# zhexin1904/gtsam_personal

Hardware: AMD Instinct MI355X
Metric: LM iterations/sec (higher is better)
Workload: dtype f64; 1 GPU; synthetic BAL 1000 cameras / 100000 points / 1000002 factors (GeneralSFMFactor<Cal3Bundler> + 2 priors), seed 42, METIS ordering (Ordering::Metis of the reference, fixture-carried permutation), LM legacy defaults; ordering=metis, cameras=1000, points=100000, factors=1000002, fronts=100001, parallelism=single GPU

## Files before the change

### gtsam_personal_amd/_lib.py

```python
from __future__ import annotations

import ctypes as ct
import os

_HERE = os.path.dirname(os.path.abspath(__file__))
LIB_PATH = os.path.join(_HERE, "liblmgpu.so")

LMGPU_OK, LMGPU_INDETERMINATE, LMGPU_INVALID, LMGPU_HIP_ERROR = 0, 1, 2, 3


class lmgpu_config(ct.Structure):
    _fields_ = [("device", ct.c_int32), ("rank", ct.c_int32), ("world_size", ct.c_int32), ("flags", ct.c_int32)]


class lmgpu_lm_params(ct.Structure):
    _fields_ = [
        ("maxIterations", ct.c_int32),
        ("relativeErrorTol", ct.c_double), ("absoluteErrorTol", ct.c_double), ("errorTol", ct.c_double),
        ("lambdaInitial", ct.c_double), ("lambdaFactor", ct.c_double), ("lambdaUpperBound", ct.c_double), ("lambdaLowerBound", ct.c_double),
        ("minModelFidelity", ct.c_double),
        ("diagonalDamping", ct.c_int32), ("useFixedLambdaFactor", ct.c_int32),
        ("minDiagonal", ct.c_double), ("maxDiagonal", ct.c_double),
    ]

# ... 119 lines not shown
    "lmgpu_ncg_optimize": (ct.c_int, [_H, ct.POINTER(lmgpu_ncg_params), ct.POINTER(lmgpu_lm_state)]),
    "lmgpu_ncg_get_trace": (ct.c_int, [_H, ct.c_int32, _D]),
    "lmgpu_ncg_host_waits": (ct.c_int, [_H]),
    "lmgpu_init_pose3_create": (ct.c_int, [ct.POINTER(lmgpu_config), ct.POINTER(_H)]),
    "lmgpu_init_pose3_destroy": (ct.c_int, [_H]),
    "lmgpu_init_pose3_last_error": (ct.c_char_p, [_H]),
    "lmgpu_init_pose3_add_factors": (ct.c_int, [_H, ct.c_int32, ct.c_int32, _I, ct.POINTER(ct.c_uint64), _D, ct.c_int32, _D]),
    "lmgpu_init_pose3_finalize": (ct.c_int, [_H, ct.c_int32, ct.POINTER(ct.c_uint64)]),
    "lmgpu_init_pose3_num_poses": (ct.c_int, [_H]),
    "lmgpu_init_pose3_num_factors": (ct.c_int, [_H]),
    "lmgpu_init_pose3_get_slots": (ct.c_int, [_H, ct.POINTER(ct.c_uint64)]),
    "lmgpu_init_pose3_handle": (ct.c_void_p, [_H, ct.c_int32]),
    "lmgpu_init_pose3_orientations_chordal": (ct.c_int, [_H, _D]),
    "lmgpu_init_pose3_closest_rotations": (ct.c_int, [ct.c_int32, ct.c_int32, _D, _D]),
    "lmgpu_init_pose3_orientations_gradient": (ct.c_int, [_H, _D, ct.c_int32, ct.c_int32, _D, _I, _D]),
    "lmgpu_init_pose3_compute_poses": (ct.c_int, [_H, _D, ct.c_int32, _D, ct.POINTER(lmgpu_lm_state)]),
    "lmgpu_init_pose3_initialize": (ct.c_int, [_H, _D, ct.c_int32, _D]),
    "lmgpu_set_kernel_timing": (ct.c_int, [_H, ct.c_int32]),
    "lmgpu_get_kernel_times": (ct.c_int, [_H, _D, _D, ct.POINTER(ct.c_int64)]),
    "lmgpu_get_jacobian": (ct.c_int, [_H, ct.c_int32, _D, _I, _I]),
    "lmgpu_get_jacobians": (ct.c_int, [_H, _I, _I, _I, _I, ct.POINTER(ct.c_int64), _D]),
    "lmgpu_num_fronts": (ct.c_int, [_H]),
    "lmgpu_front_info": (ct.c_int, [_H, ct.c_int32, _I]),
    "lmgpu_get_front": (ct.c_int, [_H, ct.c_int32, _I, _D]),
    "lmgpu_comm_unique_id": (ct.c_int, [ct.c_char_p]),
    "lmgpu_comm_init": (ct.c_int, [_H, ct.c_char_p]),
    "lmgpu_marginal_covariance": (ct.c_int, [_H, ct.c_int32, _D]),
    "lmgpu_joint_marginal_covariance": (ct.c_int, [_H, ct.c_int32, _I, _D]),
    "lmgpu_selftest_chain_schedule": (ct.c_int, [ct.c_int, ct.c_int, ct.c_int, ct.c_int, ct.c_int]),
    "lmgpu_selftest_dense_schedule": (ct.c_int, [ct.c_int, ct.c_int, ct.c_int, ct.c_uint, ct.c_int, _I]),
    "lmgpu_selftest_dogleg_step": (ct.c_int, [ct.c_int, _D, _D]),
    "lmgpu_bt_products": (ct.c_int, [_H, _D, ct.c_double, _D, _D]),
    "lmgpu_isam2_create": (ct.c_int, [ct.POINTER(lmgpu_config), ct.c_void_p, ct.c_void_p, ct.c_void_p, ct.POINTER(_H)]),
    "lmgpu_isam2_destroy": (ct.c_int, [_H]),
    "lmgpu_isam2_last_error": (ct.c_char_p, [_H]),
    "lmgpu_isam2_last_failed_key": (ct.c_uint64, [_H]),
    "lmgpu_isam2_add_variables": (ct.c_int, [_H, ct.c_int32, ct.POINTER(ct.c_uint64), _I, _D]),
    "lmgpu_isam2_add_factors": (ct.c_int, [_H, ct.c_int32, ct.c_int32, ct.POINTER(ct.c_uint64), _D, ct.c_int32, _D]),
    "lmgpu_isam2_add_factors_robust": (ct.c_int, [_H, ct.c_int32, ct.c_int32, ct.POINTER(ct.c_uint64), _D, ct.c_int32, _D, ct.c_int32, ct.c_double]),
    "lmgpu_isam2_update": (ct.c_int, [_H, ct.c_int32, ct.c_void_p]),
    "lmgpu_isam2_update_with": (ct.c_int, [_H, ct.c_void_p, ct.c_void_p]),
    "lmgpu_isam2_set_relinearize_thresholds": (ct.c_int, [_H, ct.c_int32, ct.c_char_p, _I, _D]),
    "lmgpu_isam2_set_partial_relinearization_check": (ct.c_int, [_H, ct.c_int32]),
    "lmgpu_isam2_set_dogleg": (ct.c_int, [_H, ct.c_double, ct.c_double, ct.c_int32]),
    "lmgpu_isam2_get_dogleg_delta": (ct.c_double, [_H]),
    "lmgpu_isam2_set_evaluate_nonlinear_error": (ct.c_int, [_H, ct.c_int32]),
# ... 80 lines not shown
```

### gtsam_personal_amd/csrc/kernels_front.hpp

```cpp
#pragma once
#include <hip/hip_runtime.h>

#include "kernels_factors.hpp"

namespace lmgpu {

struct FrontFac {
  int32_t fac;
  int32_t c0, c1, c2;
};
struct ChildRef {
  int64_t u_off;
  int32_t ld, m;
  int32_t map_begin;
  int32_t pad;
};
struct FrontDesc {
  int32_t n, nf;
  int32_t fac_begin, fac_count;
  int32_t child_begin, child_count;
  int32_t fx_begin;
  int32_t sx_begin;
  int64_t rsd_off;
  int64_t u_off;
// ... 1064 lines not shown
  __shared__ int s_ticket, s_ok;
  const int tid = threadIdx.x, lane = tid & 63;
  if (tid == 0) s_ticket = (int)atomicAdd(ticket, 1u);
  __syncthreads();
  const int fi = list[seg_end - 1 - s_ticket];
  const FrontDesc F = fronts[fi];
  const int ns = F.n - F.nf - 1;
  const int so = sxoff[F.sx_begin + max(min(tid, ns - 1), 0)], fo = fxoff[F.fx_begin + min(tid, F.nf - 1)];
  ldsb_stage(F, pool, Ls, tid);
  bool bad, timed_out = false;
  const double* y = ldsb_solve_core<true>(F, Ls, ns > 0 ? so : fo, delta, &bad, &timed_out);
  if (tid < F.nf)
    __hip_atomic_store((unsigned long long*)(delta + fo), (unsigned long long)__double_as_longlong(y[tid]), __ATOMIC_RELAXED, __HIP_MEMORY_SCOPE_AGENT);
  if (bad && lane == 0) atomicMin(status, F.id);
  if (timed_out) atomicExch(status + 1, 1 + F.id);
  (void)s_ok;
  (void)parent_of;
  (void)pos_of;
  (void)done;
  (void)lane;
}

}
```

### gtsam_personal_amd/csrc/lmgpu.hip

```cpp
#include <hip/hip_runtime.h>
#include <rccl/rccl.h>

#include <algorithm>
#include <chrono>
#include <cmath>
#include <cstdio>
#include <cstdlib>
#include <cstring>
#include <condition_variable>
#include <limits>
#include <mutex>
#include <string>
#include <map>
#include <vector>

#include "../../include/lmgpu.h"
#include "kernels_dense.hpp"
#include "kernels_potrf.hpp"
#include "kernels_step.hpp"
#include "dense_schedule.hpp"
#include "dogleg_step.hpp"
#include "kernels_batched.hpp"
#include "kernels_level.hpp"
#include "kernels_bayes.hpp"
// ... 33 lines not shown
  } while (0)

namespace {

struct Bucket {
  int type = 0, n = 0, noise_kind = 0;
  int robust = 0;
  double robust_k = 0.0;
  std::vector<int32_t> graph_index, slots;
  std::vector<double> meas, noise;
  int rows = 0, cols = 0;
  int n_loc = 0;
  std::vector<int32_t> loc_of;
  int64_t joff = 0;
  int32_t* d_vidx = nullptr;
  double* d_meas = nullptr;
  double* d_noise = nullptr;
  int32_t* d_epos = nullptr;
};

struct LevelWork {
  int list_begin = 0, list_count = 0;
  int lds_nf_max = 0;
  int lds_rsd_max = 0;
  int bin_begin[16] = {0};
  int bin_srows[16] = {0};
  int bin_jcap[16] = {0};
  int64_t pack_off[16] = {0};
  int pack_stride[16] = {0};
  std::vector<int> hbm;
  int small_begin = 0, small_count = 0;
  int bsd_begin = 0, bsd_count = 0;
  int med_begin = 0, med_count = 0, med_max_fac = 0, med_max_child = 0, med_max_nf = 0, med_max_cols = 0, med_max_n = 0;
  int fuse_task_begin = 0, fuse_task_count = 0, fuse_nmax = 0, fuse_jcap = 0, fuse_threads = 0;
};

struct KTimer {
  bool on = false;
  bool dominant_only = false;
  std::vector<hipEvent_t> pool;
  struct Rec {
    int cat, e0, e1, launches;
  };
  std::vector<Rec> recs;
  int used = 0;
  double ms[LMGPU_KT_NUM] = {0}, work[LMGPU_KT_NUM] = {0};
  long long cnt[LMGPU_KT_NUM] = {0};
  int grab() {
    if (used == (int)pool.size()) {
      hipEvent_t e;
      (void)hipEventCreate(&e);
      pool.push_back(e);
// ... 106 lines not shown
  int chain_split_pct = 60;
  bool chain_merge = true;
  int chain_far_pct = 50;
  double* d_lambda = nullptr;
  bool merge_backsub = false;
  struct ElimSeg {
    int lvl_lo, lvl_hi, nmax, jcap, threads;
  };
  std::vector<ElimSeg> elim_segs;
  std::vector<int> elim_seg_of;
  bool merge_elim = false;
  FillUpper* d_fill_upper = nullptr;
  int n_fill_upper = 0;
  bool fuse_levels = false;
  LevelTask* d_level_tasks = nullptr;
  LevelSync* d_level_sync = nullptr;
  int n_level_sync = 0;
  int32_t *d_bs_parent = nullptr, *d_bs_pos = nullptr;
  char* d_leafpack = nullptr;
  unsigned int* d_bs_done = nullptr;
  bool use_graph = false;
  int eager_solves = 0;
  hipGraphExec_t solve_graph[2] = {nullptr, nullptr};
  bool no_wide16 = false;
  int wide16_max = 256;
  bool bsd_ticket = false;
  bool no_tail = false;
  bool no_chain = false;
  int chain_forms = 0;
  unsigned int* d_pflags = nullptr;
  int pflags_panels = 0;
  unsigned int* bs_flags = nullptr;
  double* pool = nullptr;
  size_t pool_doubles = 0;
  double* vals[2][kNumVarTypes] = {};
  double* saved[kNumVarTypes] = {};
  int cur = 0;
  int32_t* type_xoff[kNumVarTypes] = {};
  double *delta = nullptr, *dampw = nullptr, *hdiag = nullptr, *ebuf0 = nullptr, *ebuf1 = nullptr, *partial = nullptr, *dscal = nullptr,
         *ywork = nullptr;
  int* d_status = nullptr;
  double* h_scal = nullptr;
  int* h_status = nullptr;
  FacDesc* d_fd = nullptr;
  FrontDesc* d_fronts = nullptr;
  FrontFac* d_ffac = nullptr;
// ... 494 lines not shown
    if (fused) {
      const MedLevel ML{(const MedFront*)(h->d_med_fronts + L.med_begin)};
      const size_t lds = std::max<size_t>(kLdsFrontExtra - (size_t)(LDSF_JCAP - L.fuse_jcap) * 8 + 64 + (size_t)L.fuse_nmax * L.fuse_nmax * sizeof(double),
                                          (size_t)DIAG_LDS_BYTES);
      unsigned int* ticket = h->d_bs_done + h->h_fronts.size() + li;
      const int kt = h->kt.begin(LMGPU_KT_PANEL, s);
      const bool wide = L.fuse_threads == 1024;
      auto* kernel = wide ? level_fused_kernel<1024> : level_fused_kernel<256>;
      hipLaunchKernelGGL(kernel, dim3(L.fuse_task_count), dim3(wide ? 1024 : 256), lds, s, (const LevelTask*)(h->d_level_tasks + L.fuse_task_begin), ticket,
                         (const int32_t*)h->d_lists, (const FrontDesc*)h->d_fronts, (const FrontFac*)h->d_ffac, (const FacDesc*)h->d_fd,
                         (const ChildRef*)h->d_childs, (const int32_t*)h->d_cmap, (const int32_t*)h->d_fxoff, h->pool, lambda_v, lambda_p,
                         (const double*)h->dampw, h->d_status, L.fuse_nmax, L.fuse_jcap, (const double*)h->gex_active, ML, (const int32_t*)h->d_rowptr,
                         (const RowSrc*)h->d_rowsrc, h->inv16_med, h->d_level_sync + L.med_begin);
      h->kt.end(kt, s);
    }
    for (int b = 0; b < kNumBins && seg == -1 && !fused; b++) {
      const int cnt = L.bin_begin[b + 1] - L.bin_begin[b];
      if (cnt == 0) continue;
      const int nmax = kBinN[b % 6], srows = L.bin_srows[b];
      const int threads = (b >= 6 || b % 6 == 0) ? 64 : (b % 6 == 1 ? 128 : 256);
      const int jcap = L.bin_jcap[b];
      const size_t lds = kLdsFrontExtra - (size_t)(LDSF_JCAP - jcap) * 8 + 64 + (size_t)srows * nmax * sizeof(double);
      const int kt = h->kt.begin(LMGPU_KT_LDS_FRONT, s);
      const bool wide16 = b >= 3 && b < 6 && cnt <= h->wide16_max && !h->no_wide16;
      auto* kernel = lds_front_kernel<false, 1024>;
      if (!wide16) kernel = b < 6 ? lds_front_kernel<false> : lds_front_kernel<true>;
      hipLaunchKernelGGL(kernel, dim3(cnt), dim3(wide16 ? 1024 : threads), lds, s,
                         (const int32_t*)(h->d_lists + L.list_begin + L.bin_begin[b]), (const FrontDesc*)h->d_fronts,
                         (const FrontFac*)h->d_ffac, (const FacDesc*)h->d_fd, (const ChildRef*)h->d_childs, (const int32_t*)h->d_cmap,
                         (const int32_t*)h->d_fxoff, h->pool, lambda_v, lambda_p, (const double*)h->dampw, h->d_status, nmax, srows, h->d_gcorner, jcap,
                         (const double*)h->gex_active, (const char*)(h->d_leafpack && L.pack_stride[b] ? h->d_leafpack + L.pack_off[b] : nullptr),
                         L.pack_stride[b]);
      h->kt.end(kt, s);
    }
    if (L.med_count > 0 && !fused) {
      const MedLevel ML{(const MedFront*)(h->d_med_fronts + L.med_begin)};
      const unsigned cnt = (unsigned)L.med_count;
      int ktm = h->kt.begin(LMGPU_KT_HBM_ASSEMBLE, s);
      if (L.med_max_fac > 0 || L.med_max_child > 0)
        hipLaunchKernelGGL(med_assemble_rows_kernel, dim3((L.med_max_n + 3) / 4, cnt), dim3(256), 0, s, ML, (const int32_t*)h->d_rowptr, (const RowSrc*)h->d_rowsrc, (const ChildRef*)h->d_childs, (const int32_t*)h->d_cmap,
                           (const FrontFac*)h->d_ffac, (const FacDesc*)h->d_fd, h->pool, (const int32_t*)h->d_fxoff, lambda_v, lambda_p,
                           (const double*)h->dampw, (const double*)h->gex_active);
      else
        hipLaunchKernelGGL(med_damp_kernel, dim3((L.med_max_nf + 255) / 256, cnt), dim3(256), 0, s, ML, (const int32_t*)h->d_fxoff, h->pool, lambda_v,
                           lambda_p, (const double*)h->dampw, (const double*)h->gex_active);
      h->kt.end(ktm, s);
// ... 145 lines not shown
          }
          case DENSE_TAIL: {
            const int ktt = h->kt.begin(LMGPU_KT_PANEL, s);
            hipLaunchKernelGGL(front_tail_kernel, dim3(1), dim3(256), TAIL_LDS_BYTES, s, A, ld, F.n, F.nf, k0, kb, F.id, h->d_status,
                               h->inv16 + (size_t)(i + 1) * 4096);
            h->kt.end(ktt, s, st.flop);
            break;
          }
          case DENSE_ADD_CHUNK:
          case DENSE_WAIT_CHUNK: {
            const int rcc = st.kind == DENSE_ADD_CHUNK ? add_chunk(h, A, Asm, F.n, ld, st.chunk) : wait_chunk(h, Asm, F.n, ld, st.chunk);
            if (rcc) return rcc;
            break;
          }
        }
      }
      if (run_launches > 0) h->kt.end(kt_run, s, run_flop, run_launches);
    }
  }
  HIPCHECK(hipGetLastError());
  return LMGPU_OK;
}

static bool level_lds_class(const lmgpu_handle* h, int l, int* nmax, int* jcap, int* threads) {
  const int kMergeCap = 160;
  const LevelWork& L = h->levels[l];
  if (L.list_count == 0 || L.list_count > kMergeCap || L.bin_begin[kNumBins] != L.bin_begin[6]) return false;
  int top = -1, jc = 96, cnt_top = 0;
  for (int b = 0; b < 6; b++)
    if (L.bin_begin[b + 1] > L.bin_begin[b]) {
      top = b;
      cnt_top = L.bin_begin[b + 1] - L.bin_begin[b];
      jc = std::max(jc, L.bin_jcap[b]);
    }
  *nmax = kBinN[top];
  *jcap = jc;
  const bool wide16 = top >= 3 && cnt_top <= h->wide16_max && !h->no_wide16;
  *threads = wide16 ? 1024 : (top == 0 ? 64 : 256);
  return true;
}

int do_backsub(lmgpu_handle* h) {
  hipStream_t s = h->stream;
  if (h->cfg.world_size > 1) HIPCHECK(hipMemsetAsync(h->delta, 0, h->ntot * sizeof(double), s));
  const bool merge = h->merge_backsub && h->cfg.world_size == 1 && !(h->cfg.flags & LMGPU_FLAG_SPLIT_ROOT);
  const bool no_bsd_runs = dev_switch("LMGPU_NO_BSD_RUNS") != nullptr;
  const int NFR = (int)h->h_fronts.size();
  if (h->n_fill_backsub < 0 || h->fill_backsub_merge != (int)merge) {
    std::vector<FillChunk> fills;
    if (merge) {
      add_fill(fills, h->d_bs_done, (size_t)(NFR + h->levels.size() + 1) * sizeof(unsigned int), 0u);
      add_fill(fills, h->delta, h->ntot * sizeof(double), 0xffffffffu);
    }
    if (h->bsd_x_count > 0) {
      add_fill(fills, h->d_bsd_x, h->bsd_x_count * sizeof(double), 0xffffffffu);
      add_fill(fills, h->d_bsd_ticket, h->levels.size() * sizeof(unsigned int), 0u);
    }
    if (h->d_fill_backsub) {
      HIPCHECK(hipStreamSynchronize(s));
      (void)hipFree(h->d_fill_backsub);
      h->d_fill_backsub = nullptr;
    }
    h->n_fill_backsub = (int)fills.size();
    h->fill_backsub_merge = (int)merge;
    if (!fills.empty()) {
      const int rcu = upload(h, &h->d_fill_backsub, fills);
      if (rcu) return rcu;
    }
  }
  if (h->n_fill_backsub > 0) hipLaunchKernelGGL(fill_chunks_kernel, dim3(h->n_fill_backsub), dim3(256), 0, s, (const FillChunk*)h->d_fill_backsub);
  int seg_hi = -1, seg_lo = -1;
  auto run_level = [&](const LevelWork& L) {
    if (L.lds_nf_max > LDSB_SMALL_NF) {
      hipLaunchKernelGGL(lds_backsub_wide_kernel, dim3(L.list_count), dim3(256), (size_t)(L.lds_rsd_max + LDSB_TAIL) * sizeof(double), s,
                         (const int32_t*)(h->d_lists + L.list_begin), L.list_count, (const FrontDesc*)h->d_fronts, (const int32_t*)h->d_fxoff,
                         (const int32_t*)h->d_sxoff, (const double*)h->pool, h->delta, h->d_status);
    } else {
      hipLaunchKernelGGL(lds_backsub_kernel, dim3((L.list_count + 3) / 4), dim3(256), 0, s, (const int32_t*)(h->d_lists + L.list_begin),
                         L.list_count, (const FrontDesc*)h->d_fronts, (const int32_t*)h->d_fxoff, (const int32_t*)h->d_sxoff,
                         (const double*)h->pool, h->delta, h->d_status);
    }
  };
  auto flush_segment = [&]() -> int {
    if (seg_hi < 0) return LMGPU_OK;
    const int kt = h->kt.begin(LMGPU_KT_BACKSUB_LDS, s);
    if (seg_hi == seg_lo) {
      run_level(h->levels[seg_hi]);
    } else {
      const int b = h->levels[seg_lo].list_begin, e = h->levels[seg_hi].list_begin + h->levels[seg_hi].list_count;
      int rsdmax = 0;
      for (int l = seg_lo; l <= seg_hi; l++) rsdmax = std::max(rsdmax, h->levels[l].lds_rsd_max);
      hipLaunchKernelGGL(lds_backsub_merged_kernel, dim3(e - b), dim3(256), (size_t)(rsdmax + LDSB_TAIL) * sizeof(double), s, (const int32_t*)h->d_lists, b, e,
                         (const FrontDesc*)h->d_fronts, (const int32_t*)h->d_fxoff, (const int32_t*)h->d_sxoff, (const double*)h->pool, h->delta,
                         h->d_status, (const int32_t*)h->d_bs_parent, (const int32_t*)h->d_bs_pos, h->d_bs_done, h->d_bs_done + NFR + seg_hi);
    }
    h->kt.end(kt, s);
    seg_hi = seg_lo = -1;
    return LMGPU_OK;
  };
// ... 732 lines not shown
    const Front& fr = P.fronts[fi];
    if (rep[fi]) continue;
    h->front_owner[fi] = (fr.parent < 0 || rep[fr.parent]) ? top_owner[fi] : h->front_owner[fr.parent];
  }
  for (int fi = 0; fi < NF; fi++) h->front_active[fi] = rep[fi] || h->front_owner[fi] == R;
}

}

extern "C" {

int lmgpu_create(const lmgpu_config* cfg, lmgpu_handle** out) {
  if (!cfg || !out) return LMGPU_INVALID;
  lmgpu_handle* h = new lmgpu_handle();
  h->cfg = *cfg;
  if (h->cfg.world_size < 1) h->cfg.world_size = 1;
  h->device = cfg->device;
  h->two_launch_panel = dev_switch("LMGPU_PANEL_2L") != nullptr;
  h->no_fuse = dev_switch("LMGPU_NO_FUSE") != nullptr;
  h->no_chain = dev_switch("LMGPU_NO_CHAIN") != nullptr;
  h->chain_forms = (dev_switch("LMGPU_CHAIN_FENCED_TILES") ? CHAIN_FORM_FENCED_TILES : 0) | (dev_switch("LMGPU_CHAIN_PREREAD") ? CHAIN_FORM_PREREAD : 0);
  h->no_tail = dev_switch("LMGPU_NO_TAIL") != nullptr;
  h->no_wide16 = dev_switch("LMGPU_NO_WIDE16") != nullptr;
  if (const char* e = dev_switch("LMGPU_WIDE16_MAX")) h->wide16_max = atoi(e);
  h->bsd_ticket = dev_switch("LMGPU_BSD_TICKET") != nullptr;
  h->no_gather_write = dev_switch("LMGPU_NO_GATHER_WRITE") != nullptr;
  h->schur_split_diag = dev_switch("LMGPU_SCHUR_SPLIT_DIAG") != nullptr;
  h->pcg_fused = dev_switch("LMGPU_PCG_FUSED") != nullptr;
  if (dev_switch("LMGPU_NO_MERGE")) h->chain_merge = false;
  if (const char* e = dev_switch("LMGPU_CHAIN_SPLIT")) h->chain_split_pct = std::max(0, std::min(100, atoi(e)));
  if (const char* e = dev_switch("LMGPU_CHAIN_FAR")) h->chain_far_pct = std::max(10, std::min(100, atoi(e)));
  *out = h;
  if (h->device >= 0) {
    HIPCHECK(hipSetDevice(h->device));
    {
      hipDeviceProp_t prop;
      HIPCHECK(hipGetDeviceProperties(&prop, h->device));
      h->num_cus = prop.multiProcessorCount;
    }
    HIPCHECK(hipStreamCreate(&h->stream));
    {
      int prio_lo = 0, prio_hi = 0;
      HIPCHECK(hipDeviceGetStreamPriorityRange(&prio_lo, &prio_hi));
      HIPCHECK(hipStreamCreateWithPriority(&h->comm_stream, hipStreamNonBlocking, prio_hi));
    }
    HIPCHECK(hipEventCreateWithFlags(&h->asm_ev, hipEventDisableTiming));
// ... 593 lines not shown
  std::vector<int32_t> lists;
  for (int l = 0; l < P.n_levels; l++) {
    LevelWork& L = h->levels[l];
    L.list_begin = (int)lists.size();
    int c = 0;
    for (int b = 0; b < kNumBins; b++) {
      L.bin_begin[b] = c;
      L.bin_srows[b] = kBinN[b % 6];
      if (b >= 6) {
        int mx = 1;
        for (int fi : byLevelBin[l][b]) mx = std::max(mx, P.fronts[fi].nf);
        L.bin_srows[b] = mx;
      }
      int jc = 96;
      for (int fi : byLevelBin[l][b]) {
        int tot = 0;
        for (int32_t f : P.fronts[fi].factors) tot += fd[h->fac_local[f]].rows * (fd[h->fac_local[f]].d0 + fd[h->fac_local[f]].d1 + fd[h->fac_local[f]].d2 + 1);
        jc = std::max(jc, std::min(tot, LDSF_JCAP));
      }
      L.bin_jcap[b] = (jc + 7) & ~7;
      for (int fi : byLevelBin[l][b]) {
        lists.push_back(fi);
        L.lds_nf_max = std::max(L.lds_nf_max, (int)P.fronts[fi].nf);
        L.lds_rsd_max = std::max(L.lds_rsd_max, (int)P.fronts[fi].nf * ((int)P.fronts[fi].n | 1));
      }
      c += (int)byLevelBin[l][b].size();
    }
    L.bin_begin[kNumBins] = c;
    L.list_count = c;
  }
  {
    h->elim_segs.clear();
    h->elim_seg_of.assign(P.n_levels, -1);
    auto level_class = [&](int l, int* nmax, int* jcap, int* threads) { return level_lds_class(h, l, nmax, jcap, threads); };
    int l = 0;
    while (l < P.n_levels) {
      int nmax, jcap, threads;
      if (!level_class(l, &nmax, &jcap, &threads)) {
        l++;
        continue;
      }
      lmgpu_handle::ElimSeg E{l, l, nmax, jcap, threads};
      while (E.lvl_hi + 1 < P.n_levels && h->levels[E.lvl_hi].hbm.empty()) {
        int n2, j2, t2;
        if (!level_class(E.lvl_hi + 1, &n2, &j2, &t2) || (t2 == 1024) != (E.threads == 1024)) break;
        E.lvl_hi++;
        E.nmax = std::max(E.nmax, n2);
        E.jcap = std::max(E.jcap, j2);
        E.threads = std::max(E.threads, t2);
      }
      if (E.lvl_hi > E.lvl_lo) {
        h->elim_seg_of[E.lvl_lo] = (int)h->elim_segs.size();
        for (int q = E.lvl_lo + 1; q <= E.lvl_hi; q++) h->elim_seg_of[q] = -2;
// ... 1183 lines not shown
  std::vector<std::vector<double>> jb(h->buckets.size());
  for (size_t k = 0; k < h->buckets.size(); k++) {
    const Bucket& b = h->buckets[k];
    jb[k].resize((size_t)b.n_loc * b.rows * b.cols);
    if (b.n_loc) HIPCHECK(hipMemcpy(jb[k].data(), h->pool + b.joff, jb[k].size() * sizeof(double), hipMemcpyDeviceToHost));
  }
  off = 0;
  for (int i = 0; i < NFAC; i++) {
    const FactorRef& f = h->plan.factors[i];
    const Bucket& b = h->buckets[f.bucket];
    const size_t sz = (size_t)b.rows * b.cols;
    if (b.loc_of[f.idx] < 0) {
      h->err = "lmgpu_get_jacobians: a factor lives on another rank";
      return LMGPU_INVALID;
    }
    std::memcpy(out + off, jb[f.bucket].data() + (size_t)b.loc_of[f.idx] * sz, sz * sizeof(double));
    off += (int64_t)sz;
  }
  return LMGPU_OK;
}

int lmgpu_num_fronts(const lmgpu_handle* h) { return (h && h->finalized) ? (int)h->plan.fronts.size() : -1; }

int lmgpu_front_info(const lmgpu_handle* h, int32_t front, int32_t* info) {
  if (!h || !h->finalized || front < 0 || front >= (int)h->plan.fronts.size() || !info) return LMGPU_INVALID;
  const Front& fr = h->plan.fronts[front];
  info[0] = (int)fr.vars.size();
  info[1] = fr.n_frontal_vars;
  info[2] = fr.nf;
  info[3] = fr.n;
  info[4] = fr.parent;
  info[5] = fr.cls;
  info[6] = h->front_owner[front];
  info[7] = fr.level;
  return LMGPU_OK;
}

int lmgpu_get_front(lmgpu_handle* h, int32_t front, int32_t* slots, double* RSd) {
  if (!h) return LMGPU_INVALID;
  if (!h->finalized || front < 0 || front >= (int)h->plan.fronts.size()) {
    h->err = "lmgpu_get_front: refused (!h->finalized || front < 0 || front >= (int)h->plan.fronts.size())";
    return LMGPU_INVALID;
  }
  const Front& fr = h->plan.fronts[front];
  if (slots) std::memcpy(slots, fr.vars.data(), fr.vars.size() * sizeof(int32_t));
  if (RSd) {
// ... 382 lines not shown
```

### gtsam_personal_amd/optimizer.py

```python
from __future__ import annotations

import ctypes as ct

import numpy as np

from . import _lib
from .graph import (CAM_BUNDLER, F_PRIOR_CAM, F_SFM, FACTOR_ARITY, N_UNIT, VAR_DIM, VAR_STORE, VAR_STORE_DEV, NonlinearFactorGraph, Ordering,
                    Values)


class DummyPreconditionerParameters:
    kind = _lib.LMGPU_PRECOND_DUMMY


class BlockJacobiPreconditionerParameters:
    kind = _lib.LMGPU_PRECOND_BLOCK_JACOBI


class PCGSolverParameters:

    def __init__(self, preconditioner=None):
        self.minIterations = 1
        self.maxIterations = 500
        self.reset = 501
# ... 302 lines not shown

    def hessian_diagonal(self):
        d = np.empty(self._ntot)
        self._check(self.lib.lmgpu_hessian_diagonal(self._h, _dp(d)))
        return self.delta_by_key(d)

    def bt_products(self, x=None, alpha=0.0):
        g, sq = np.empty(self._ntot), ct.c_double()
        xp = None if x is None else np.ascontiguousarray(x, dtype=np.float64)
        assert xp is None or xp.shape == (self._ntot,)
        self._check(self.lib.lmgpu_bt_products(self._h, None if xp is None else _dp(xp), float(alpha), ct.byref(sq), _dp(g)))
        return (None if xp is None else sq.value), g

    def jacobian(self, graph_index):
        r, c = ct.c_int32(), ct.c_int32()
        self._check(self.lib.lmgpu_get_jacobian(self._h, graph_index, None, ct.byref(r), ct.byref(c)))
        out = np.empty(r.value * c.value)
        self._check(self.lib.lmgpu_get_jacobian(self._h, graph_index, _dp(out), ct.byref(r), ct.byref(c)))
        return out.reshape(c.value, r.value).T.copy()

    def num_fronts(self):
        return self.lib.lmgpu_num_fronts(self._h)

    def front_info(self, i):
        info = np.zeros(8, dtype=np.int32)
        self._check(self.lib.lmgpu_front_info(self._h, i, _ip(info)))
        return dict(n_keys=int(info[0]), n_frontal_keys=int(info[1]), nf=int(info[2]), n=int(info[3]), parent=int(info[4]), cls=int(info[5]),
                    owner=int(info[6]), level=int(info[7]))

    def front(self, i, numeric=True):
        fi = self.front_info(i)
        slots = np.zeros(fi["n_keys"], dtype=np.int32)
        rsd = np.empty(fi["nf"] * fi["n"]) if numeric else None
        self._check(self.lib.lmgpu_get_front(self._h, i, _ip(slots), _dp(rsd) if numeric else None))
        keys = [int(self._keys[s]) for s in slots]
        return keys, (rsd.reshape(fi["n"], fi["nf"]).T.copy() if numeric else None)


class JacobianFactor:

    def __init__(self, keys, dims, Ab):
        self._keys, self._dims, self._Ab = list(keys), list(dims), Ab
        self._off = np.concatenate([[0], np.cumsum(dims)]).astype(int)

    def keys(self):
        return list(self._keys)
# ... 428 lines not shown
```

### include/lmgpu.h

```cpp
#ifndef LMGPU_H
#define LMGPU_H
#include <stdint.h>

#ifdef __cplusplus
extern "C" {
#endif

typedef struct lmgpu_handle lmgpu_handle;

enum lmgpu_status {
  LMGPU_OK = 0,
  LMGPU_INDETERMINATE = 1,
  LMGPU_INVALID = 2,
  LMGPU_HIP_ERROR = 3
};

enum lmgpu_var_type {
  LMGPU_POSE2 = 0,
  LMGPU_POSE3 = 1,
  LMGPU_POINT3 = 2,
  LMGPU_CAM_BUNDLER = 3,
  LMGPU_POINT2 = 4,
  LMGPU_CAL3_S2 = 5,
  LMGPU_VEC9 = 6,
// ... 175 lines not shown
int lmgpu_init_pose3_initialize(lmgpu_init_pose3* ip, const double* guess_R, int32_t use_gradient, double* poses_out);

enum lmgpu_kernel_category {
  LMGPU_KT_LINEARIZE = 0,
  LMGPU_KT_LDS_FRONT = 1,
  LMGPU_KT_HBM_ASSEMBLE = 2,
  LMGPU_KT_PANEL = 3,
  LMGPU_KT_SYRK = 4,
  LMGPU_KT_BACKSUB_HBM = 5,
  LMGPU_KT_BACKSUB_LDS = 6,
  LMGPU_KT_LINEAR_ERROR = 7,
  LMGPU_KT_RETRACT_ERROR = 8,
  LMGPU_KT_ALLREDUCE = 9,
  LMGPU_KT_CHAIN = 10,
  LMGPU_KT_NUM = 11
};
int lmgpu_set_kernel_timing(lmgpu_handle* h, int32_t on);
int lmgpu_get_kernel_times(const lmgpu_handle* h, double* ms , double* work , int64_t* launches );

int lmgpu_get_jacobian(lmgpu_handle* h, int32_t graph_index, double* out, int32_t* rows, int32_t* cols);
int lmgpu_get_jacobians(lmgpu_handle* h, int32_t* n_out, int32_t* graph_index, int32_t* rows, int32_t* cols, int64_t* offsets, double* out);
int lmgpu_num_fronts(const lmgpu_handle* h);
int lmgpu_front_info(const lmgpu_handle* h, int32_t front, int32_t* info8);
int lmgpu_get_front(lmgpu_handle* h, int32_t front, int32_t* slots, double* RSd_colmajor);

int lmgpu_comm_unique_id(char id128[128]);
int lmgpu_comm_init(lmgpu_handle* h, const char id128[128]);

int lmgpu_marginal_covariance(lmgpu_handle* h, int32_t slot, double* cov );
int lmgpu_joint_marginal_covariance(lmgpu_handle* h, int32_t nslots, const int32_t* slots, double* cov );

int lmgpu_selftest_chain_schedule(int n, int nf, int i0, int nsteps, int far_pct);

int lmgpu_selftest_dense_schedule(int n, int nf, int mode, unsigned forms, int max_records, int32_t* out);

int lmgpu_selftest_dogleg_step(int which, const double* in, double* out);

typedef struct lmgpu_isam2 lmgpu_isam2;
typedef int (*lmgpu_ccolamd_fn)(void* user, int32_t n_rows, int32_t n_cols, const int32_t* col_ptr, const int32_t* row_idx, const int32_t* cmember,
                                int32_t* perm_out);
typedef struct lmgpu_isam2_params {
  double relinearizeThreshold;
  int32_t relinearizeSkip;
  int32_t enableRelinearization;
  double wildfireThreshold;
} lmgpu_isam2_params;
// ... 66 lines not shown
```

Measured before the change: 137.9 LM iterations/s.

## Factor tiny leaf fronts with 16-lane groups using DPP reductions

Adds a grouped leaf-front kernel that maps each small leaf front (nf<=4, up to 32 small factors) onto a 16-lane sub-group. It builds the Hessian via register-level DPP reductions, runs an in-register Cholesky and writes the RSd and separator update blocks. It also adds a matching 16-lane grouped back-substitution kernel for levels whose fronts have tiny frontal blocks. The goal is to replace one-block-per-front or few-fronts-per-block processing of the ~100k point fronts, which wastes threads and LDS, with much denser packing. This comes at the cost of heavy template register pressure and new numerical and eligibility paths.

```diff
diff --git a/gtsam_personal_amd/_lib.py b/gtsam_personal_amd/_lib.py
--- a/gtsam_personal_amd/_lib.py
+++ b/gtsam_personal_amd/_lib.py
@@ -165,6 +165,9 @@
     "lmgpu_get_jacobians": (ct.c_int, [_H, _I, _I, _I, _I, ct.POINTER(ct.c_int64), _D]),
     "lmgpu_num_fronts": (ct.c_int, [_H]),
     "lmgpu_front_info": (ct.c_int, [_H, ct.c_int32, _I]),
+    "lmgpu_leaf_group_launches": (ct.c_int, [_H]),
+    "lmgpu_backsub_group_launches": (ct.c_int, [_H, _I]),
+    "lmgpu_get_leaf_corner": (ct.c_int, [_H, ct.c_int32, _D]),
     "lmgpu_get_front": (ct.c_int, [_H, ct.c_int32, _I, _D]),
     "lmgpu_comm_unique_id": (ct.c_int, [ct.c_char_p]),
     "lmgpu_comm_init": (ct.c_int, [_H, ct.c_char_p]),
diff --git a/gtsam_personal_amd/csrc/kernels_front.hpp b/gtsam_personal_amd/csrc/kernels_front.hpp
--- a/gtsam_personal_amd/csrc/kernels_front.hpp
+++ b/gtsam_personal_amd/csrc/kernels_front.hpp
@@ -1110,3 +1110,5 @@
 }
 
 }
+
+#include "kernels_leaf.hpp"
diff --git a/gtsam_personal_amd/csrc/kernels_leaf.hpp b/gtsam_personal_amd/csrc/kernels_leaf.hpp
--- /dev/null
+++ b/gtsam_personal_amd/csrc/kernels_leaf.hpp
@@ -0,0 +1,306 @@
+#pragma once
+
+namespace lmgpu {
+
+#define LEAFGRP_MAXNF 4
+#define LEAFGRP_MAXROWS 4
+#define LEAFGRP_MAXSEP 9
+#define LEAFGRP_LANES 16
+
+template <int CTRL>
+__device__ __forceinline__ double leafgrp_dpp(double v) {
+  const long long b = __double_as_longlong(v);
+  const int lo = __builtin_amdgcn_update_dpp(0, (int)(b & 0xffffffffLL), CTRL, 0xf, 0xf, false);
+  const int hi = __builtin_amdgcn_update_dpp(0, (int)(b >> 32), CTRL, 0xf, 0xf, false);
+  return __longlong_as_double(((long long)hi << 32) | (unsigned int)lo);
+}
+__device__ __forceinline__ double leafgrp_sum16(double v) {
+  v += leafgrp_dpp<0xB1>(v);
+  v += leafgrp_dpp<0x4E>(v);
+  v += leafgrp_dpp<0x141>(v);
+  v += leafgrp_dpp<0x140>(v);
+  return v;
+}
+
+template <int MR, int DS, int NFM>
+struct LeafGrpFac {
+  double af[MR][NFM];
+  double b[MR];
+  double as[MR][DS];
+  int cs, ds;
+};
+template <int MR, int DS, int NFM, bool WITH_SEP, bool FIRST>
+__device__ __forceinline__ void leafgrp_load(LeafGrpFac<MR, DS, NFM>& G, const LFac* __restrict__ lf, int f, int nfac, int nf, const double* stage,
+                                             double (&H)[NFM][NFM], double (&g)[NFM], double& cc) {
+  constexpr int NF = NFM, XR = LEAFGRP_MAXROWS - MR;
+  const bool act = f < nfac;
+  const LFac d = lf[min(f, nfac - 1)];
+  const double* J = stage + d.off;
+  const int m = d.rows;
+  const bool f0 = d.c0 < nf;
+  const int qf = f0 ? 0 : d.d0, df = f0 ? d.d0 : d.d1, cf = f0 ? d.c0 : d.c1;
+  const int qs = f0 ? d.d0 : 0;
+  G.ds = (act && d.d1 > 0) ? (f0 ? d.d1 : d.d0) : 0;
+  G.cs = f0 ? d.c1 : d.c0;
+  const int qb = d.d0 + d.d1;
+  double xa[XR > 0 ? XR : 1][NF], xb[XR > 0 ? XR : 1];
+#pragma unroll
+  for (int r = 0; r < LEAFGRP_MAXROWS; r++) {
+#pragma unroll
+    for (int I = 0; I < NF; I++) {
+      const double v = (act && r < m && I >= cf && I < cf + df) ? J[(qf + I - cf) * m + r] : 0.0;
+      if (r < MR)
+        G.af[r][I] = v;
+      else
+        xa[r - MR][I] = v;
+    }
+    const double v = (act && r < m) ? J[qb * m + r] : 0.0;
+    if (r < MR)
+      G.b[r] = v;
+    else
+      xb[r - MR] = v;
+  }
+  if constexpr (WITH_SEP) {
+#pragma unroll
+    for (int r = 0; r < MR; r++)
+#pragma unroll
+      for (int c = 0; c < DS; c++) G.as[r][c] = (r < m && c < G.ds) ? J[(qs + c) * m + r] : 0.0;
+  }
+#pragma unroll
+  for (int I = 0; I < NF; I++) {
+#pragma unroll
+    for (int Jc = I; Jc <= NF; Jc++) {
+      double v = 0.0;
+#pragma unroll
+      for (int r = 0; r < MR; r++) v += G.af[r][I] * (Jc < NF ? G.af[r][Jc] : G.b[r]);
+#pragma unroll
+      for (int r = 0; r < XR; r++) v += xa[r][I] * (Jc < NF ? xa[r][Jc] : xb[r]);
+      double& dst = Jc < NF ? H[I][Jc] : g[I];
+      dst = FIRST ? v : dst + v;
+    }
+  }
+  double v = 0.0;
+#pragma unroll
+  for (int r = 0; r < MR; r++) v += G.b[r] * G.b[r];
+#pragma unroll
+  for (int r = 0; r < XR; r++) v += xb[r] * xb[r];
+  cc = FIRST ? v : cc + v;
+}
+
+template <int MR, int DS, int NFM>
+__global__ __launch_bounds__(256) __attribute__((amdgpu_waves_per_eu(NFM <= 3 ? 4 : 2, NFM <= 3 ? 4 : 2))) void lds_front_group_kernel(const char* __restrict__ pack, int pack_stride, int nleaf, double* __restrict__ pool, double lambda_v,
+                                                               const double* __restrict__ lambda_p, const double* __restrict__ dampw, int* __restrict__ status,
+                                                               double* __restrict__ gcorner, const double* __restrict__ gex, int lds_leaf, int out_off) {
+  extern __shared__ double leafgrp_lds[];
+  constexpr int NF = NFM;
+  const int tid = threadIdx.x, gl = tid & (LEAFGRP_LANES - 1);
+  const int leaf = (int)(blockIdx.x * blockDim.x + tid) / LEAFGRP_LANES;
+  const bool live = leaf < nleaf;
+  const char* pk = pack + (size_t)min(leaf, nleaf - 1) * pack_stride;
+  const FrontDesc F = *(const FrontDesc*)pk;
+  const int nfac = ((const int*)(pk + LEAFPACK_HDR))[0], tot = ((const int*)(pk + LEAFPACK_HDR))[1], contig = ((const int*)(pk + LEAFPACK_HDR))[2];
+  const LFac* lf = (const LFac*)(pk + LEAFPACK_FAC);
+  const int n = F.n, nf = F.nf;
+  const double lambda = lambda_p ? *lambda_p : lambda_v;
+  double dw[NF];
+#pragma unroll
+  for (int i = 0; i < NF; i++) dw[i] = dampw[((const int*)(pk + LEAFPACK_XO))[min(i, nf - 1)]];
+  double* stage = leafgrp_lds + (size_t)(tid / LEAFGRP_LANES) * lds_leaf;
+  double* X = stage + out_off;
+  if (contig) {
+    const double* J = pool + lf[0].joff;
+    for (int i0 = gl; i0 < tot; i0 += 16 * LEAFGRP_LANES) {
+      double v[16];
+#pragma unroll
+      for (int u = 0; u < 16; u++) v[u] = J[min(i0 + u * LEAFGRP_LANES, tot - 1)];
+#pragma unroll
+      for (int u = 0; u < 16; u++)
+        if (i0 + u * LEAFGRP_LANES < tot) stage[i0 + u * LEAFGRP_LANES] = v[u];
+    }
+  } else {
+    for (int f = 0; f < nfac; f++) {
+      const LFac d = lf[f];
+      const double* J = pool + d.joff;
+      for (int i = gl; i < d.sz; i += LEAFGRP_LANES) stage[d.off + i] = J[i];
+    }
+  }
+  __syncthreads();
+  LeafGrpFac<MR, DS, NFM> G;
+  double H[NF][NF], g[NF], cc;
+  leafgrp_load<MR, DS, NFM, true, true>(G, lf, gl, nfac, nf, stage, H, g, cc);
+  if (nfac > LEAFGRP_LANES) {
+    LeafGrpFac<MR, DS, NFM> G2;
+    leafgrp_load<MR, DS, NFM, false, false>(G2, lf, gl + LEAFGRP_LANES, nfac, nf, stage, H, g, cc);
+  }
+#pragma unroll
+  for (int I = 0; I < NF; I++) {
+#pragma unroll
+    for (int J = I; J < NF; J++) H[I][J] = leafgrp_sum16(H[I][J]);
+    g[I] = leafgrp_sum16(g[I]);
+  }
+  cc = leafgrp_sum16(cc);
+#pragma unroll
+  for (int I = 0; I < NF; I++) {
+    if (I < nf) {
+      H[I][I] += lambda * dw[I];
+      if (gex) g[I] += gex[((const int*)(pk + LEAFPACK_XO))[I]];
+    } else {
+      H[I][I] = 1.0;
+    }
+  }
+  bool failed = false;
+  double inv[NF];
+#pragma unroll
+  for (int k = 0; k < NF; k++) {
+    double piv = H[k][k];
+    if (!(piv > 0.0)) {
+      if (piv <= 0.0) failed = true;
+      piv = (piv == piv && piv != 0.0) ? fabs(piv) : 1.0;
+    }
+    const double r = sqrt(piv);
+    inv[k] = 1.0 / r;
+    H[k][k] = r;
+#pragma unroll
+    for (int J = k + 1; J < NF; J++) H[k][J] *= inv[k];
+    g[k] *= inv[k];
+    cc -= g[k] * g[k];
+#pragma unroll
+    for (int I = k + 1; I < NF; I++) {
+#pragma unroll
+      for (int J = I; J < NF; J++) H[I][J] -= H[k][I] * H[k][J];
+      g[I] -= H[k][I] * g[k];
+    }
+  }
+  {
+    double dlast = H[0][0], dprev = H[0][0];
+#pragma unroll
+    for (int I = 1; I < NF; I++)
+      if (I < nf) {
+        dprev = dlast;
+        dlast = H[I][I];
+      }
+    if (nf >= 2) {
+      if (!(frexp_exp(dprev) - frexp_exp(dlast) < 12)) failed = true;
+    } else {
+      if (!(frexp_exp(dlast) > -12)) failed = true;
+    }
+  }
+  if (live && gl == 0) {
+    if (failed) atomicMin(status, F.id);
+    gcorner[F.par_map] = cc;
+  }
+  if (gl < nf) {
+    double row[NF], di = g[0];
+#pragma unroll
+    for (int J = 0; J < NF; J++) row[J] = H[0][J];
+#pragma unroll
+    for (int I = 1; I < NF; I++)
+      if (gl == I) {
+        di = g[I];
+#pragma unroll
+        for (int J = 0; J < NF; J++) row[J] = J >= I ? H[I][J] : 0.0;
+      }
+#pragma unroll
+    for (int J = 0; J < NF; J++)
+      if (J < nf) X[gl * n + J] = row[J];
+    X[gl * n + n - 1] = di;
+  }
+  auto emit = [&](const LeafGrpFac<MR, DS, NFM>& Q) {
+#pragma unroll
+    for (int c = 0; c < DS; c++) {
+      double s[NF];
+#pragma unroll
+      for (int I = 0; I < NF; I++) {
+        double v = 0.0;
+#pragma unroll
+        for (int r = 0; r < MR; r++) v += Q.af[r][I] * Q.as[r][c];
+        s[I] = v;
+      }
+#pragma unroll
+      for (int k = 0; k < NF; k++) {
+        s[k] *= inv[k];
+#pragma unroll
+        for (int I = k + 1; I < NF; I++) s[I] -= H[k][I] * s[k];
+      }
+      if (c < Q.ds) {
+#pragma unroll
+        for (int I = 0; I < NF; I++)
+          if (I < nf) X[I * n + Q.cs + c] = s[I];
+      }
+    }
+  };
+  emit(G);
+  if (nfac > LEAFGRP_LANES) {
+    double H2[NF][NF], g2[NF], c2;
+    leafgrp_load<MR, DS, NFM, true, true>(G, lf, gl + LEAFGRP_LANES, nfac, nf, stage, H2, g2, c2);
+    emit(G);
+  }
+  __syncthreads();
+  if (live) {
+    double* RSd = pool + F.rsd_off;
+    double* St = pool + F.u_off;
+    const int nx = nf * n, nt = (n - nf) * nf;
+    for (int i = gl; i < nx; i += LEAFGRP_LANES) RSd[i] = X[i];
+    for (int i = gl; i < nt; i += LEAFGRP_LANES) {
+      const int c = nf == 3 ? (int)(((unsigned)i * 43691u) >> 17) : (nf == 1 ? i : i >> (nf >> 1));
+      St[i] = X[(i - c * nf) * n + nf + c];
+    }
+  }
+}
+
+#define LDSBG_MAXNF 4
+template <int NFM, int NQ>
+__global__ __launch_bounds__(256) void lds_backsub_group_kernel(const int32_t* __restrict__ list, int nlist, const FrontDesc* __restrict__ fronts,
+                                                                 const int32_t* __restrict__ fxoff, const int32_t* __restrict__ sxoff,
+                                                                 const double* __restrict__ pool, double* __restrict__ delta, int* __restrict__ status) {
+  const int tid = threadIdx.x, gl = tid & (LEAFGRP_LANES - 1);
+  const int li = (int)(blockIdx.x * blockDim.x + tid) / LEAFGRP_LANES;
+  const bool live = li < nlist;
+  const FrontDesc F = fronts[list[min(li, nlist - 1)]];
+  const int n = F.n, nf = F.nf, ns = n - nf - 1;
+  const double* RSd = pool + F.rsd_off;
+  const int fo = fxoff[F.fx_begin + min(gl, nf - 1)];
+  int so[NQ];
+#pragma unroll
+  for (int q = 0; q < NQ; q++) so[q] = ns > 0 ? sxoff[F.sx_begin + min(gl + LEAFGRP_LANES * q, ns - 1)] : 0;
+  double sv[NFM][NQ], R[NFM][NFM], rhs[NFM];
+#pragma unroll
+  for (int u = 0; u < NFM; u++) {
+    const double* row = RSd + (size_t)min(u, nf - 1) * F.ld_rsd;
+#pragma unroll
+    for (int q = 0; q < NQ; q++) sv[u][q] = row[nf + max(min(gl + LEAFGRP_LANES * q, ns - 1), 0)];
+#pragma unroll
+    for (int k = 0; k < NFM; k++) R[u][k] = row[min(k, nf - 1)];
+    rhs[u] = row[n - 1];
+  }
+  double xs[NQ];
+#pragma unroll
+  for (int q = 0; q < NQ; q++) {
+    const double v = delta[so[q]];
+    xs[q] = (gl + LEAFGRP_LANES * q < ns) ? v : 0.0;
+  }
+#pragma unroll
+  for (int u = 0; u < NFM; u++) {
+    double acc = sv[u][0] * xs[0];
+#pragma unroll
+    for (int q = 1; q < NQ; q++) acc += sv[u][q] * xs[q];
+    rhs[u] -= leafgrp_sum16(acc);
+  }
+  double x[NFM];
+#pragma unroll
+  for (int k = NFM - 1; k >= 0; k--) {
+    double t = rhs[k];
+#pragma unroll
+    for (int j = k + 1; j < NFM; j++) t -= (j < nf ? R[k][j] : 0.0) * x[j];
+    x[k] = k < nf ? t / R[k][k] : 0.0;
+  }
+  double xi = x[0];
+#pragma unroll
+  for (int k = 1; k < NFM; k++) xi = gl == k ? x[k] : xi;
+  if (live && gl < nf) {
+    delta[fo] = xi;
+    if (xi != xi) atomicMin(status, F.id);
+  }
+}
+
+}
diff --git a/gtsam_personal_amd/csrc/lmgpu.hip b/gtsam_personal_amd/csrc/lmgpu.hip
--- a/gtsam_personal_amd/csrc/lmgpu.hip
+++ b/gtsam_personal_amd/csrc/lmgpu.hip
@@ -79,12 +79,15 @@
 struct LevelWork {
   int list_begin = 0, list_count = 0;
   int lds_nf_max = 0;
+  int lds_ns_max = 0;
   int lds_rsd_max = 0;
   int bin_begin[16] = {0};
   int bin_srows[16] = {0};
   int bin_jcap[16] = {0};
   int64_t pack_off[16] = {0};
   int pack_stride[16] = {0};
+  uint8_t bin_group[16] = {0};
+  int bin_group_out[16] = {0}, bin_group_maxfac[16] = {0};
   std::vector<int> hbm;
   int small_begin = 0, small_count = 0;
   int bsd_begin = 0, bsd_count = 0;
@@ -237,6 +240,9 @@
   bool use_graph = false;
   int eager_solves = 0;
   hipGraphExec_t solve_graph[2] = {nullptr, nullptr};
+  int leaf_group_threads = 256;
+  bool no_backsub_groups = false;
+  int n_leaf_group_launches = 0;
   bool no_wide16 = false;
   int wide16_max = 256;
   bool bsd_ticket = false;
@@ -777,6 +783,19 @@
       const int jcap = L.bin_jcap[b];
       const size_t lds = kLdsFrontExtra - (size_t)(LDSF_JCAP - jcap) * 8 + 64 + (size_t)srows * nmax * sizeof(double);
       const int kt = h->kt.begin(LMGPU_KT_LDS_FRONT, s);
+      if (L.bin_group[b]) {
+        auto* gk = L.bin_group[b] == 1 ? lds_front_group_kernel<2, LEAFGRP_MAXSEP, 3> : lds_front_group_kernel<LEAFGRP_MAXROWS, LEAFGRP_MAXSEP, LEAFGRP_MAXNF>;
+        const int out_off = L.bin_group_maxfac[b] > LEAFGRP_LANES ? jcap : 0;
+        const int lds_leaf = (std::max(jcap, out_off + L.bin_group_out[b]) + 1) & ~1;
+        int gthreads = h->leaf_group_threads;
+        while (gthreads > 64 && (size_t)(gthreads / LEAFGRP_LANES) * lds_leaf * sizeof(double) > 65536) gthreads >>= 1;
+        const int lpw = gthreads / LEAFGRP_LANES;
+        hipLaunchKernelGGL(gk, dim3((cnt + lpw - 1) / lpw), dim3(gthreads), (size_t)lpw * lds_leaf * sizeof(double), s,
+                           (const char*)(h->d_leafpack + L.pack_off[b]), L.pack_stride[b], cnt, h->pool, lambda_v,
+                           lambda_p, (const double*)h->dampw, h->d_status, h->d_gcorner, (const double*)h->gex_active, lds_leaf, out_off);
+        h->kt.end(kt, s);
+        continue;
+      }
       const bool wide16 = b >= 3 && b < 6 && cnt <= h->wide16_max && !h->no_wide16;
       auto* kernel = lds_front_kernel<false, 1024>;
       if (!wide16) kernel = b < 6 ? lds_front_kernel<false> : lds_front_kernel<true>;
@@ -968,6 +987,34 @@
   return LMGPU_OK;
 }
 
+static int leaf_group_form(const FrontDesc& F, const FrontFac* ffac, const FacDesc* fd, int jcap) {
+  if (F.par_ld != -1 || F.pad != 0 || F.nf < 1 || F.nf > LEAFGRP_MAXNF || F.nf > LEAFPACK_MAXNF || F.ld_rsd != F.n) return 0;
+  if (F.fac_count < 1 || F.fac_count > LDSF_MAXB) return 0;
+  int form = F.nf <= 3 ? 1 : 2, tot = 0;
+  int32_t seen[LDSF_MAXB];
+  int nseen = 0;
+  for (int k = 0; k < F.fac_count; k++) {
+    const FrontFac& ff = ffac[F.fac_begin + k];
+    const FacDesc& d = fd[ff.fac];
+    tot += d.rows * (d.d0 + d.d1 + d.d2 + 1);
+    if (d.d2 > 0 || d.rows < 1 || d.rows > LEAFGRP_MAXROWS) return 0;
+    if (d.d1 == 0) {
+      if (ff.c0 + d.d0 > F.nf) return 0;
+      continue;
+    }
+    const bool f0 = ff.c0 < F.nf, f1 = ff.c1 < F.nf;
+    if (f0 == f1) return 0;
+    const int cf = f0 ? ff.c0 : ff.c1, df = f0 ? d.d0 : d.d1, cs = f0 ? ff.c1 : ff.c0, ds = f0 ? d.d1 : d.d0;
+    if (cf + df > F.nf || ds > LEAFGRP_MAXSEP || cs + ds > F.n - 1) return 0;
+    for (int q = 0; q < nseen; q++)
+      if (seen[q] == cs) return 0;
+    seen[nseen++] = cs;
+    if (d.rows > 2) form = 2;
+  }
+  if (tot > jcap) return 0;
+  return form;
+}
+
 static bool level_lds_class(const lmgpu_handle* h, int l, int* nmax, int* jcap, int* threads) {
   const int kMergeCap = 160;
   const LevelWork& L = h->levels[l];
@@ -984,6 +1031,11 @@
   const bool wide16 = top >= 3 && cnt_top <= h->wide16_max && !h->no_wide16;
   *threads = wide16 ? 1024 : (top == 0 ? 64 : 256);
   return true;
+}
+
+static int backsub_group_form(const lmgpu_handle* h, const LevelWork& L) {
+  if (L.list_count == 0 || L.lds_nf_max > LDSBG_MAXNF || h->no_backsub_groups) return 0;
+  return (L.lds_nf_max <= 3 && L.lds_ns_max <= 6 * LEAFGRP_LANES) ? 1 : 2;
 }
 
 int do_backsub(lmgpu_handle* h) {
@@ -1021,6 +1073,11 @@
       hipLaunchKernelGGL(lds_backsub_wide_kernel, dim3(L.list_count), dim3(256), (size_t)(L.lds_rsd_max + LDSB_TAIL) * sizeof(double), s,
                          (const int32_t*)(h->d_lists + L.list_begin), L.list_count, (const FrontDesc*)h->d_fronts, (const int32_t*)h->d_fxoff,
                          (const int32_t*)h->d_sxoff, (const double*)h->pool, h->delta, h->d_status);
+    } else if (const int form = backsub_group_form(h, L)) {
+      auto* gk = form == 1 ? lds_backsub_group_kernel<3, 6> : lds_backsub_group_kernel<LDSBG_MAXNF, 9>;
+      hipLaunchKernelGGL(gk, dim3((L.list_count + 15) / 16), dim3(256), 0, s, (const int32_t*)(h->d_lists + L.list_begin), L.list_count,
+                         (const FrontDesc*)h->d_fronts, (const int32_t*)h->d_fxoff, (const int32_t*)h->d_sxoff, (const double*)h->pool, h->delta,
+                         h->d_status);
     } else {
       hipLaunchKernelGGL(lds_backsub_kernel, dim3((L.list_count + 3) / 4), dim3(256), 0, s, (const int32_t*)(h->d_lists + L.list_begin),
                          L.list_count, (const FrontDesc*)h->d_fronts, (const int32_t*)h->d_fxoff, (const int32_t*)h->d_sxoff,
@@ -1799,6 +1856,8 @@
   h->chain_forms = (dev_switch("LMGPU_CHAIN_FENCED_TILES") ? CHAIN_FORM_FENCED_TILES : 0) | (dev_switch("LMGPU_CHAIN_PREREAD") ? CHAIN_FORM_PREREAD : 0);
   h->no_tail = dev_switch("LMGPU_NO_TAIL") != nullptr;
   h->no_wide16 = dev_switch("LMGPU_NO_WIDE16") != nullptr;
+  if (const char* e = dev_switch("LMGPU_LEAF_GROUP_THREADS")) h->leaf_group_threads = atoi(e) == 64 ? 64 : (atoi(e) == 128 ? 128 : 256);
+  h->no_backsub_groups = dev_switch("LMGPU_NO_BACKSUB_GROUPS") != nullptr;
   if (const char* e = dev_switch("LMGPU_WIDE16_MAX")) h->wide16_max = atoi(e);
   h->bsd_ticket = dev_switch("LMGPU_BSD_TICKET") != nullptr;
   h->no_gather_write = dev_switch("LMGPU_NO_GATHER_WRITE") != nullptr;
@@ -2438,6 +2497,7 @@
       for (int fi : byLevelBin[l][b]) {
         lists.push_back(fi);
         L.lds_nf_max = std::max(L.lds_nf_max, (int)P.fronts[fi].nf);
+        L.lds_ns_max = std::max(L.lds_ns_max, (int)P.fronts[fi].n - (int)P.fronts[fi].nf - 1);
         L.lds_rsd_max = std::max(L.lds_rsd_max, (int)P.fronts[fi].nf * ((int)P.fronts[fi].n | 1));
       }
       c += (int)byLevelBin[l][b].size();
@@ -2445,6 +2505,22 @@
     L.bin_begin[kNumBins] = c;
     L.list_count = c;
   }
+  h->n_leaf_group_launches = 0;
+  if (!dev_switch("LMGPU_NO_LEAF_GROUPS") && !dev_switch("LMGPU_NO_LEAFPACK") && !h->pcg_structure)
+    for (LevelWork& L : h->levels)
+      for (int b = 6; b < kNumBins; b++) {
+        const int cnt = L.bin_begin[b + 1] - L.bin_begin[b];
+        int form = cnt > 0 ? 1 : 0;
+        for (int q = 0; q < cnt && form; q++) {
+          const FrontDesc& F = h->h_fronts[lists[L.list_begin + L.bin_begin[b] + q]];
+          const int f = leaf_group_form(F, ffac.data(), fd.data(), L.bin_jcap[b]);
+          form = f ? std::max(form, f) : 0;
+          L.bin_group_out[b] = std::max(L.bin_group_out[b], F.nf * F.n);
+          L.bin_group_maxfac[b] = std::max(L.bin_group_maxfac[b], F.fac_count);
+        }
+        L.bin_group[b] = (uint8_t)form;
+        if (form) h->n_leaf_group_launches++;
+      }
   {
     h->elim_segs.clear();
     h->elim_seg_of.assign(P.n_levels, -1);
@@ -3674,6 +3750,34 @@
 
 int lmgpu_num_fronts(const lmgpu_handle* h) { return (h && h->finalized) ? (int)h->plan.fronts.size() : -1; }
 
+int lmgpu_leaf_group_launches(const lmgpu_handle* h) { return (h && h->finalized) ? h->n_leaf_group_launches : -1; }
+
+int lmgpu_backsub_group_launches(const lmgpu_handle* h, int32_t* wide) {
+  if (!h || !h->finalized) return -1;
+  int cnt = 0, w = 0;
+  for (const LevelWork& L : h->levels) {
+    const int form = backsub_group_form(h, L);
+    cnt += form != 0;
+    w += form == 2;
+  }
+  if (wide) *wide = w;
+  return cnt;
+}
+
+int lmgpu_get_leaf_corner(lmgpu_handle* h, int32_t front, double* corner) {
+  if (!h) return LMGPU_INVALID;
+  if (!h->finalized || front < 0 || front >= (int)h->plan.fronts.size() || !corner) {
+    h->err = "lmgpu_get_leaf_corner: refused (!h->finalized || front < 0 || front >= (int)h->plan.fronts.size() || !corner)";
+    return LMGPU_INVALID;
+  }
+  int rc = need_device(h);
+  if (rc) return rc;
+  const FrontDesc& F = h->h_fronts[front];
+  if (!h->solved || !h->front_active[front] || F.par_ld != -1 || !h->d_gcorner) return LMGPU_INVALID;
+  HIPCHECK(hipMemcpy(corner, h->d_gcorner + F.par_map, sizeof(double), hipMemcpyDeviceToHost));
+  return LMGPU_OK;
+}
+
 int lmgpu_front_info(const lmgpu_handle* h, int32_t front, int32_t* info) {
   if (!h || !h->finalized || front < 0 || front >= (int)h->plan.fronts.size() || !info) return LMGPU_INVALID;
   const Front& fr = h->plan.fronts[front];
diff --git a/gtsam_personal_amd/optimizer.py b/gtsam_personal_amd/optimizer.py
--- a/gtsam_personal_amd/optimizer.py
+++ b/gtsam_personal_amd/optimizer.py
@@ -348,6 +348,18 @@
     def num_fronts(self):
         return self.lib.lmgpu_num_fronts(self._h)
 
+    def leaf_group_launches(self):
+        return self.lib.lmgpu_leaf_group_launches(self._h)
+
+    def backsub_group_launches(self):
+        wide = np.zeros(1, dtype=np.int32)
+        return self.lib.lmgpu_backsub_group_launches(self._h, _ip(wide)), int(wide[0])
+
+    def leaf_corner(self, i):
+        out = np.zeros(1)
+        self._check(self.lib.lmgpu_get_leaf_corner(self._h, i, _dp(out)))
+        return float(out[0])
+
     def front_info(self, i):
         info = np.zeros(8, dtype=np.int32)
         self._check(self.lib.lmgpu_front_info(self._h, i, _ip(info)))
diff --git a/include/lmgpu.h b/include/lmgpu.h
--- a/include/lmgpu.h
+++ b/include/lmgpu.h
@@ -221,6 +221,9 @@
 int lmgpu_get_jacobians(lmgpu_handle* h, int32_t* n_out, int32_t* graph_index, int32_t* rows, int32_t* cols, int64_t* offsets, double* out);
 int lmgpu_num_fronts(const lmgpu_handle* h);
 int lmgpu_front_info(const lmgpu_handle* h, int32_t front, int32_t* info8);
+int lmgpu_leaf_group_launches(const lmgpu_handle* h);
+int lmgpu_backsub_group_launches(const lmgpu_handle* h, int32_t* wide);
+int lmgpu_get_leaf_corner(lmgpu_handle* h, int32_t front, double* corner);
 int lmgpu_get_front(lmgpu_handle* h, int32_t front, int32_t* slots, double* RSd_colmajor);
 
 int lmgpu_comm_unique_id(char id128[128]);
```

Result: faster. 141.0 LM iterations/s, median of 6 (+2.2%).
